# Visual-Behavior/aloception-oss

Measured on AMD Instinct MI355X. Metric: frames/sec (whole node) DeformableDETR-R50 inference, higher is better.
Workload: dtype bf16; 1 GPU; DeformableDETR-R50 inference bf16, batch 8 synthetic 1333x800 frames per GPU, random-init weights; launch=hip-graph replay + eager inference(), per_gpu_batch=8, global_batch=8, parallelism=batch-sharded x1, no collective

## Files before the change

### aloception-oss_amd/csrc/common.hpp

```cpp
#pragma once
#include <hip/hip_runtime.h>
#include <stdint.h>

#include <cstdarg>
#include <cstdio>
#include <type_traits>

#include "../../include/alo_hotpath.h"

namespace alo {

char* error_buffer();
inline int fail(alo_status_t code, const char* fmt, ...) {
    va_list ap;
    va_start(ap, fmt);
    vsnprintf(error_buffer(), 512, fmt, ap);
    va_end(ap);
    return (int)code;
}
#define ALO_REQUIRE(cond, code, ...) \
    do {                             \
        if (!(cond)) return ::alo::fail(code, __VA_ARGS__); \
    } while (0)

template <typename... P>
inline bool aligned16(const P*... p) {
    return ((... | (uintptr_t)p) & 15) == 0;
}

constexpr int kLdsLimit = 160 * 1024;
template <auto kernel>
int launch(dim3 grid, dim3 block, size_t lds, hipStream_t stream, const char* what, void** args) {
    ALO_REQUIRE(lds <= (size_t)kLdsLimit, ALO_ERR_UNSUPPORTED, "%s: %zu bytes of dynamic LDS, the limit is %d", what, lds, kLdsLimit);
    const void* fn = reinterpret_cast<const void*>(kernel);
    hipError_t e = hipSuccess;
    if (lds > 48 * 1024) {
        static unsigned long long done = 0;
        int dev = 0;
        e = hipGetDevice(&dev);
        const unsigned long long bit = 1ull << (dev & 63);
        if (e == hipSuccess && !(__atomic_load_n(&done, __ATOMIC_ACQUIRE) & bit)) {
            e = hipFuncSetAttribute(fn, hipFuncAttributeMaxDynamicSharedMemorySize, kLdsLimit);
            if (e == hipSuccess) __atomic_fetch_or(&done, bit, __ATOMIC_RELEASE);
        }
    }
    if (e == hipSuccess) e = hipLaunchKernel(fn, grid, block, args, lds, stream);
    if (e == hipSuccess) e = hipGetLastError();
    if (e != hipSuccess) return fail(ALO_ERR_LAUNCH, "%s: %s", what, hipGetErrorString(e));
    return ALO_OK;
}

constexpr int kNumXcd = 8;

__device__ __forceinline__ unsigned xcd_contiguous_block(unsigned bid, unsigned nblocks) {
    const unsigned q = nblocks / kNumXcd, r = nblocks % kNumXcd;
    const unsigned xcd = bid % kNumXcd, k = bid / kNumXcd;
    const unsigned start = xcd < r ? xcd * (q + 1) : r * (q + 1) + (xcd - r) * q;
    return start + k;
}

struct WidePlan {
    int words[31];
};
bool msda_wide_plan(int N, int S, int M, int D, int Lq, int value_dtype, const int32_t* host_shapes, WidePlan* wp);
int msda_wide_launch(const void* value, const int32_t* shapes, const int32_t* lstart, const void* loc, const void* attn,
                     const void* grad_out, void* grad_value, void* grad_loc, void* grad_attn, const WidePlan& wp, int D,
                     int value_dtype, hipStream_t stream);

struct RowGather {
    int s, Wo, HoWo, W, HW;
};
inline RowGather row_gather(int stride = 1, int Ho = 1, int Wo = 1, int H = 1, int W = 1) { return {stride, Wo, Ho * Wo, W, H * W}; }

int linear_shortk_gather(const void* x, const void* weight, const void* bias, const void* residual, void* y, long M, int N, int K,
                         int relu, const RowGather& gather, hipStream_t stream);

#define ALO_RELU_RES(fn, first, relu, residual, ...)                                                                          \
    ((residual) ? ((relu) ? fn<first, true, true>(__VA_ARGS__) : fn<first, false, true>(__VA_ARGS__))                          \
                : ((relu) ? fn<first, true, false>(__VA_ARGS__) : fn<first, false, false>(__VA_ARGS__)))

typedef __attribute__((ext_vector_type(4))) unsigned int u32x4;
typedef __attribute__((ext_vector_type(2))) unsigned int u32x2;
typedef __attribute__((ext_vector_type(4))) float f32x4;
typedef __attribute__((ext_vector_type(16))) float f32x16;

struct bf16_t {
    uint16_t bits;
};

__device__ __forceinline__ float relu_keep_nan(float v) { return (v > 0.f || v != v) ? v : 0.f; }

__device__ __forceinline__ float bf16_to_f32(uint16_t b) { return __uint_as_float(((unsigned)b) << 16); }
__device__ __forceinline__ uint16_t f32_to_bf16(float f) {
    const __bf16 b = static_cast<__bf16>(f);
    return __builtin_bit_cast(uint16_t, b);
}
__device__ __forceinline__ unsigned pack_bf16x2(float lo, float hi) {
    typedef __bf16 bf16x2_hw __attribute__((ext_vector_type(2)));
    typedef float f32x2_hw __attribute__((ext_vector_type(2)));
    const bf16x2_hw r = __builtin_convertvector(f32x2_hw{lo, hi}, bf16x2_hw);
    return __builtin_bit_cast(unsigned, r);
}

struct f16_t {
    uint16_t bits;
};
__device__ __forceinline__ float f16_to_f32(uint16_t b) { return (float)__builtin_bit_cast(_Float16, b); }
__device__ __forceinline__ uint16_t f32_to_f16(float f) {
    const _Float16 h = static_cast<_Float16>(f);
    return __builtin_bit_cast(uint16_t, h);
}
__device__ __forceinline__ unsigned pack_f16x2(float lo, float hi) {
    typedef _Float16 f16x2_hw __attribute__((ext_vector_type(2)));
    typedef float f32x2_hw __attribute__((ext_vector_type(2)));
    const f16x2_hw r = __builtin_convertvector(f32x2_hw{lo, hi}, f16x2_hw);
    return __builtin_bit_cast(unsigned, r);
}
template <typename T>
__device__ __forceinline__ void unpack2(unsigned w, float& lo, float& hi) {
    if constexpr (std::is_same<T, f16_t>::value) {
        lo = f16_to_f32((uint16_t)(w & 0xffffu));
        hi = f16_to_f32((uint16_t)(w >> 16));
    } else {
        lo = __uint_as_float(w << 16);
        hi = __uint_as_float(w & 0xffff0000u);
    }
}
template <typename T>
__device__ __forceinline__ unsigned pack2(float lo, float hi) {
    if constexpr (std::is_same<T, f16_t>::value) return pack_f16x2(lo, hi);
    else return pack_bf16x2(lo, hi);
}

typedef __attribute__((ext_vector_type(8))) __bf16 bf16x8_t;
__device__ __forceinline__ bf16x8_t as_bf16x8(const u32x4& v) {
    union { u32x4 u; bf16x8_t b; } x;
    x.u = v;
    return x.b;
}

typedef __attribute__((ext_vector_type(8))) _Float16 f16x8_t;
__device__ __forceinline__ f16x8_t as_f16x8(const u32x4& v) {
    union { u32x4 u; f16x8_t h; } x;
    x.u = v;
    return x.h;
}
template <typename T>
__device__ __forceinline__ f32x16 mfma_32x32x16(const u32x4& a, const u32x4& b, const f32x16& c) {
    if constexpr (std::is_same<T, f16_t>::value) return __builtin_amdgcn_mfma_f32_32x32x16_f16(as_f16x8(a), as_f16x8(b), c, 0, 0, 0);
    else return __builtin_amdgcn_mfma_f32_32x32x16_bf16(as_bf16x8(a), as_bf16x8(b), c, 0, 0, 0);
}

template <typename T, bool RELU>
__device__ __forceinline__ u32x4 add_residual_x8(const u32x4& v, const u32x4& rv) {
    const unsigned a4[4] = {v.x, v.y, v.z, v.w}, r4[4] = {rv.x, rv.y, rv.z, rv.w};
    unsigned o4[4];
#pragma unroll
    for (int i = 0; i < 4; ++i) {
        float alo, ahi, rlo, rhi;
        unpack2<T>(a4[i], alo, ahi);
        unpack2<T>(r4[i], rlo, rhi);
        float lo = alo + rlo, hi = ahi + rhi;
        if (RELU) { lo = relu_keep_nan(lo); hi = relu_keep_nan(hi); }
        o4[i] = pack2<T>(lo, hi);
    }
    return u32x4{o4[0], o4[1], o4[2], o4[3]};
}

__device__ __forceinline__ long gather_row(const RowGather& g, long row) {
    if (g.s <= 1) return row;
    const long n = row / g.HoWo;
    const int rem = (int)(row - n * g.HoWo);
    const int yo = rem / g.Wo, xo = rem - yo * g.Wo;
    return n * g.HW + (long)(yo * g.s) * g.W + xo * g.s;
}

__device__ __forceinline__ __amdgpu_buffer_rsrc_t make_rsrc(const void* base, unsigned bytes) {
    return __builtin_amdgcn_make_buffer_rsrc(const_cast<void*>(base), 0, (int)bytes, 0x00020000);
}
constexpr unsigned kOutOfRange = 0xC0000000u;

template <typename T, typename CT, int VEC>
struct Loader;

template <>
struct Loader<float, float, 4> {
    using raw_t = u32x4;
    static __device__ __forceinline__ raw_t load(__amdgpu_buffer_rsrc_t r, unsigned off) {
        return __builtin_amdgcn_raw_buffer_load_b128(r, off, 0, 0);
    }
    static __device__ __forceinline__ void widen(const raw_t& x, float (&v)[4]) {
        v[0] = __uint_as_float(x.x); v[1] = __uint_as_float(x.y); v[2] = __uint_as_float(x.z); v[3] = __uint_as_float(x.w);
    }
};
template <>
struct Loader<float, float, 1> {
    using raw_t = unsigned;
    static __device__ __forceinline__ raw_t load(__amdgpu_buffer_rsrc_t r, unsigned off) {
        return __builtin_amdgcn_raw_buffer_load_b32(r, off, 0, 0);
    }
    static __device__ __forceinline__ void widen(const raw_t& x, float (&v)[1]) { v[0] = __uint_as_float(x); }
};
template <>
struct Loader<double, double, 2> {
    using raw_t = u32x4;
    static __device__ __forceinline__ raw_t load(__amdgpu_buffer_rsrc_t r, unsigned off) {
        return __builtin_amdgcn_raw_buffer_load_b128(r, off, 0, 0);
    }
    static __device__ __forceinline__ void widen(const raw_t& x, double (&v)[2]) {
        v[0] = __hiloint2double((int)x.y, (int)x.x);
        v[1] = __hiloint2double((int)x.w, (int)x.z);
    }
};
template <>
struct Loader<double, double, 1> {
    using raw_t = u32x2;
    static __device__ __forceinline__ raw_t load(__amdgpu_buffer_rsrc_t r, unsigned off) {
        return __builtin_amdgcn_raw_buffer_load_b64(r, off, 0, 0);
    }
    static __device__ __forceinline__ void widen(const raw_t& x, double (&v)[1]) {
        v[0] = __hiloint2double((int)x.y, (int)x.x);
    }
};
template <>
struct Loader<bf16_t, float, 8> {
    using raw_t = u32x4;
    static __device__ __forceinline__ raw_t load(__amdgpu_buffer_rsrc_t r, unsigned off) {
        return __builtin_amdgcn_raw_buffer_load_b128(r, off, 0, 0);
    }
    static __device__ __forceinline__ void widen(const raw_t& x, float (&v)[8]) {
        const unsigned w[4] = {x.x, x.y, x.z, x.w};
#pragma unroll
        for (int i = 0; i < 4; ++i) {
            v[2 * i] = __uint_as_float(w[i] << 16);
            v[2 * i + 1] = __uint_as_float(w[i] & 0xffff0000u);
        }
    }
};
template <>
struct Loader<bf16_t, float, 1> {
    using raw_t = unsigned short;
    static __device__ __forceinline__ raw_t load(__amdgpu_buffer_rsrc_t r, unsigned off) {
        return __builtin_amdgcn_raw_buffer_load_b16(r, off, 0, 0);
    }
    static __device__ __forceinline__ void widen(const raw_t& x, float (&v)[1]) { v[0] = bf16_to_f32(x); }
};

template <>
struct Loader<f16_t, float, 8> {
    using raw_t = u32x4;
    static __device__ __forceinline__ raw_t load(__amdgpu_buffer_rsrc_t r, unsigned off) {
        return __builtin_amdgcn_raw_buffer_load_b128(r, off, 0, 0);
    }
    static __device__ __forceinline__ void widen(const raw_t& x, float (&v)[8]) {
        const unsigned w[4] = {x.x, x.y, x.z, x.w};
#pragma unroll
        for (int i = 0; i < 4; ++i) unpack2<f16_t>(w[i], v[2 * i], v[2 * i + 1]);
    }
};
template <>
struct Loader<f16_t, float, 1> {
    using raw_t = unsigned short;
    static __device__ __forceinline__ raw_t load(__amdgpu_buffer_rsrc_t r, unsigned off) {
        return __builtin_amdgcn_raw_buffer_load_b16(r, off, 0, 0);
    }
    static __device__ __forceinline__ void widen(const raw_t& x, float (&v)[1]) { v[0] = f16_to_f32(x); }
};

__device__ __forceinline__ float ld(const float* p) { return *p; }
__device__ __forceinline__ double ld(const double* p) { return *p; }
__device__ __forceinline__ float ld(const bf16_t* p) { return bf16_to_f32(p->bits); }
__device__ __forceinline__ float ld(const f16_t* p) { return f16_to_f32(p->bits); }
__device__ __forceinline__ void st(float* p, float v) { *p = v; }
__device__ __forceinline__ void st(double* p, double v) { *p = v; }
__device__ __forceinline__ void st(bf16_t* p, float v) { p->bits = f32_to_bf16(v); }
__device__ __forceinline__ void st(f16_t* p, float v) { p->bits = f32_to_f16(v); }

template <typename T, typename CT, int VEC>
__device__ __forceinline__ void store_vec(T* p, const CT (&v)[VEC]) {
    if constexpr (sizeof(T) == 4 && VEC == 4) {
        *reinterpret_cast<f32x4*>(p) = f32x4{(float)v[0], (float)v[1], (float)v[2], (float)v[3]};
    } else if constexpr (sizeof(T) == 8 && VEC == 2) {
        *reinterpret_cast<double2*>(p) = double2{(double)v[0], (double)v[1]};
    } else if constexpr (sizeof(T) == 2 && VEC == 8) {
        u32x4 o;
        o.x = pack2<T>(v[0], v[1]);
        o.y = pack2<T>(v[2], v[3]);
        o.z = pack2<T>(v[4], v[5]);
        o.w = pack2<T>(v[6], v[7]);
        *reinterpret_cast<u32x4*>(p) = o;
    } else {
#pragma unroll
        for (int i = 0; i < VEC; ++i) st(p + i, v[i]);
    }
}

__device__ __forceinline__ float wave_sum(float v) {
#pragma unroll
    for (int o = 32; o > 0; o >>= 1) v += __shfl_xor(v, o, 64);
    return v;
}

constexpr int kTileRows = 64;
constexpr int kTileStride = 256 * 2 + 16;
constexpr int kTileKB = 2;
constexpr int kTileBatches = 16 / kTileKB;

template <typename T>
__device__ __forceinline__ void load_batch(u32x4 (&buf)[2][kTileKB], const T* frag0, size_t tile_stride, int batch) {
#pragma unroll
    for (int t = 0; t < 2; ++t)
#pragma unroll
        for (int j = 0; j < kTileKB; ++j)
            buf[t][j] = *reinterpret_cast<const u32x4*>(frag0 + t * tile_stride + (size_t)(kTileKB * batch + j) * 512);
    __builtin_amdgcn_sched_barrier(0);
}
template <typename T = bf16_t>
__device__ __forceinline__ void mma_batch(f32x16 (&acc)[2][2], const unsigned char* a_lds, const u32x4 (&buf)[2][kTileKB], int batch,
                                          int nl, int kg) {
    u32x4 af[2][kTileKB];
#pragma unroll
    for (int j = 0; j < kTileKB; ++j) {
        const int s = kTileKB * batch + j;
        af[0][j] = *reinterpret_cast<const u32x4*>(a_lds + nl * kTileStride + (16 * s + 8 * kg) * 2);
        af[1][j] = *reinterpret_cast<const u32x4*>(a_lds + (32 + nl) * kTileStride + (16 * s + 8 * kg) * 2);
    }
#pragma unroll
    for (int j = 0; j < kTileKB; ++j) {
        const u32x4 a0 = af[0][j], a1 = af[1][j];
        acc[0][0] = mfma_32x32x16<T>(buf[0][j], a0, acc[0][0]);
        acc[0][1] = mfma_32x32x16<T>(buf[1][j], a0, acc[0][1]);
        acc[1][0] = mfma_32x32x16<T>(buf[0][j], a1, acc[1][0]);
        acc[1][1] = mfma_32x32x16<T>(buf[1][j], a1, acc[1][1]);
    }
    __builtin_amdgcn_sched_barrier(0);
}
template <typename T>
__device__ __forceinline__ void mma_tile256(f32x16 (&acc)[2][2], const unsigned char* a_lds, u32x4 (&bufa)[2][kTileKB],
                                            u32x4 (&bufb)[2][kTileKB], const T* w, size_t tile_stride, const T* next,
                                            size_t next_stride, int nl, int kg) {
#pragma unroll
    for (int bt = 0; bt < kTileBatches; bt += 2) {
        load_batch(bufb, w, tile_stride, bt + 1);
        mma_batch<T>(acc, a_lds, bufa, bt, nl, kg);
        if (bt + 2 < kTileBatches) load_batch(bufa, w, tile_stride, bt + 2);
        else if (next != nullptr) load_batch(bufa, next, next_stride, 0);
        mma_batch<T>(acc, a_lds, bufb, bt + 1, nl, kg);
    }
}

template <typename T>
__device__ __forceinline__ void fetch_tile256(u32x4 (&v)[8], const T* X, long row0, long M, int tid) {
#pragma unroll
    for (int j = 0; j < 8; ++j) {
        const int p = tid + 256 * j;
        long row = row0 + (p >> 5);
        row = row < M ? row : M - 1;
        v[j] = *reinterpret_cast<const u32x4*>(X + row * 256 + (p & 31) * 8);
    }
}
__device__ __forceinline__ void park_tile256(unsigned char* lds, const u32x4 (&v)[8], int tid) {
#pragma unroll
    for (int j = 0; j < 8; ++j) {
        const int p = tid + 256 * j;
        *reinterpret_cast<u32x4*>(lds + (p >> 5) * kTileStride + (p & 31) * 16) = v[j];
    }
}
template <bool ADD_BIAS, bool RELU, typename T = bf16_t>
__device__ __forceinline__ void stage_tile256(unsigned char* lds, const f32x16 (&acc)[2][2], const float* bias, int wave, int nl, int kg) {
#pragma unroll
    for (int t = 0; t < 2; ++t)
#pragma unroll
        for (int q = 0; q < 4; ++q) {
            const int col = 64 * wave + 32 * t + 8 * q + 4 * kg;
            f32x4 bb = {0.f, 0.f, 0.f, 0.f};
            if constexpr (ADD_BIAS) bb = *reinterpret_cast<const f32x4*>(bias + col);
#pragma unroll
            for (int a = 0; a < 2; ++a) {
                float v0 = acc[a][t][4 * q], v1 = acc[a][t][4 * q + 1], v2 = acc[a][t][4 * q + 2], v3 = acc[a][t][4 * q + 3];
                if constexpr (ADD_BIAS) { v0 += bb[0]; v1 += bb[1]; v2 += bb[2]; v3 += bb[3]; }
                if constexpr (RELU) { v0 = relu_keep_nan(v0); v1 = relu_keep_nan(v1); v2 = relu_keep_nan(v2); v3 = relu_keep_nan(v3); }
                *reinterpret_cast<u32x2*>(lds + (32 * a + nl) * kTileStride + col * 2) = u32x2{pack2<T>(v0, v1), pack2<T>(v2, v3)};
            }
        }
}

}
```

### aloception-oss_amd/csrc/gemm.hip

```cpp
#include "common.hpp"

namespace alo {
namespace {

constexpr int kRows = 64;
constexpr int kOutStride = 64 * 2 + 16;

struct GemmDims {
    long M;
    int N;
    int tiles;
    int S;
    RowGather g;
};

template <typename T, int kK, bool RELU, bool HAS_RES, bool HM>
__global__ void __launch_bounds__(256, 2)
linear_shortk_kernel(const T* __restrict__ X, const T* __restrict__ W, const T* __restrict__ bias,
                     const T* __restrict__ R, T* __restrict__ Y, const GemmDims dm) {
    constexpr int kRowBytes = kK * 2 + 16;
    constexpr int kSteps = kK / 16;
    constexpr int kPieces = kK / 8;
    constexpr int kLoads = kRows * kPieces / 256;
    static_assert(kRows * kPieces % 256 == 0, "the tile loader gives every thread the same number of pieces");
    extern __shared__ __attribute__((aligned(16))) unsigned char smem[];
    unsigned char* const xbuf = smem;
    const int tid = threadIdx.x, wave = tid >> 6, lane = tid & 63;
    unsigned char* obuf = smem + kRows * kRowBytes + wave * (kRows * kOutStride);

    const int col0 = blockIdx.y * 256 + wave * 64;
    const bool has_cols = col0 < dm.N;
    const int nl = lane & 31, kg = lane >> 5;

    u32x4 wreg[2][kSteps];
    float* const bias_tab = reinterpret_cast<float*>(smem + kRows * kRowBytes + 4 * (kRows * kOutStride)) + wave * 64;
    if (has_cols) {
#pragma unroll
        for (int t = 0; t < 2; ++t) {
            const T* wr = W + (size_t)(col0 + 32 * t + nl) * kK + 8 * kg;
#pragma unroll
            for (int s = 0; s < kSteps; ++s) wreg[t][s] = *reinterpret_cast<const u32x4*>(wr + 16 * s);
        }
        const int r = lane & 15, t = (lane >> 4) & 1, k2 = lane >> 5;
        bias_tab[lane] = bias != nullptr ? ld(&bias[col0 + 32 * t + (r & 3) + 8 * (r >> 2) + 4 * k2]) : 0.f;
    }

    auto fetch = [&](int tile, u32x4 (&r)[kLoads]) {
#pragma unroll
        for (int j = 0; j < kLoads; ++j) {
            const int p = tid + 256 * j;
            long row = (long)tile * kRows + p / kPieces;
            row = gather_row(dm.g, row < dm.M ? row : dm.M - 1);
            r[j] = *reinterpret_cast<const u32x4*>(X + row * kK + (p % kPieces) * 8);
        }
    };
    auto park = [&](const u32x4 (&r)[kLoads]) {
#pragma unroll
        for (int j = 0; j < kLoads; ++j) {
            const int p = tid + 256 * j;
            *reinterpret_cast<u32x4*>(xbuf + (p / kPieces) * kRowBytes + (p % kPieces) * 16) = r[j];
        }
    };

    int tile = blockIdx.x;
    if (tile >= dm.tiles) return;
    u32x4 stage[kLoads];
    fetch(tile, stage);

    for (;;) {
        park(stage);
        __syncthreads();
        const int next = tile + gridDim.x;
        const bool more = next < dm.tiles;
        if (more) fetch(next, stage);

        if (has_cols) {
#pragma unroll
            for (int half = 0; half < kRows / 32; ++half) {
                f32x16 acc[2];
#pragma unroll
                for (int t = 0; t < 2; ++t)
#pragma unroll
                    for (int q = 0; q < 4; ++q) {
                        const f32x4 b4 = *reinterpret_cast<const f32x4*>(bias_tab + (kg * 2 + t) * 16 + 4 * q);
#pragma unroll
                        for (int i = 0; i < 4; ++i) acc[t][4 * q + i] = b4[i];
                    }
#pragma unroll
                for (int s = 0; s < kSteps; ++s) {
                    const u32x4 a = *reinterpret_cast<const u32x4*>(xbuf + (32 * half + nl) * kRowBytes + (16 * s + 8 * kg) * 2);
                    acc[0] = mfma_32x32x16<T>(wreg[0][s], a, acc[0]);
                    acc[1] = mfma_32x32x16<T>(wreg[1][s], a, acc[1]);
                }
#pragma unroll
                for (int t = 0; t < 2; ++t)
#pragma unroll
                    for (int q = 0; q < 4; ++q) {
                        float v0 = acc[t][4 * q], v1 = acc[t][4 * q + 1], v2 = acc[t][4 * q + 2], v3 = acc[t][4 * q + 3];
                        if (RELU && !HAS_RES) { v0 = relu_keep_nan(v0); v1 = relu_keep_nan(v1); v2 = relu_keep_nan(v2); v3 = relu_keep_nan(v3); }
                        *reinterpret_cast<u32x2*>(obuf + (32 * half + nl) * kOutStride + (32 * t + 8 * q + 4 * kg) * 2) =
                            u32x2{pack2<T>(v0, v1), pack2<T>(v2, v3)};
                    }
            }
            __builtin_amdgcn_fence(__ATOMIC_RELEASE, "wavefront");
            __builtin_amdgcn_wave_barrier();
            __builtin_amdgcn_fence(__ATOMIC_ACQUIRE, "wavefront");
            if constexpr (HM) {
                const unsigned char* mask = reinterpret_cast<const unsigned char*>(R);
                const int heads = dm.N / 32;
#pragma unroll
                for (int hh = 0; hh < 2; ++hh) {
#pragma unroll
                    for (int pass = 0; pass < kRows / 16; ++pass) {
                        const int row = pass * 16 + (lane >> 2);
                        const long grow = (long)tile * kRows + row;
                        if (grow < dm.M) {
                            u32x4 v = *reinterpret_cast<const u32x4*>(obuf + row * kOutStride + hh * 64 + (lane & 3) * 16);
                            if (mask != nullptr && mask[grow]) v = u32x4{0u, 0u, 0u, 0u};
                            const long nb = grow / dm.S, sp = grow - nb * dm.S;
                            const int head = col0 / 32 + hh;
                            *reinterpret_cast<u32x4*>(Y + ((nb * heads + head) * dm.S + sp) * 32 + (lane & 3) * 8) = v;
                        }
                    }
                }
            } else
#pragma unroll
            for (int pass = 0; pass < kRows / 8; ++pass) {
                const int row = pass * 8 + (lane >> 3);
                const long grow = (long)tile * kRows + row;
                u32x4 v = *reinterpret_cast<const u32x4*>(obuf + row * kOutStride + (lane & 7) * 16);
                if (grow < dm.M) {
                    if constexpr (HAS_RES) {
                        v = add_residual_x8<T, RELU>(v, *reinterpret_cast<const u32x4*>(R + grow * dm.N + col0 + (lane & 7) * 8));
                    }
                    *reinterpret_cast<u32x4*>(Y + grow * dm.N + col0 + (lane & 7) * 8) = v;
                }
            }
        }
        if (!more) break;
        __syncthreads();
        tile = next;
    }
}

}
}

using namespace alo;

namespace {
template <typename T, int kK>
struct ShortK {
    using type = T;
    static constexpr int K = kK;
};

template <class Cfg, bool RELU, bool HAS_RES, bool HM = false>
int launch_shortk(const void* x, const void* weight, const void* bias, const void* residual, void* y, long M, int N,
                  hipStream_t stream, int S = 0, const RowGather& gather = row_gather()) {
    GemmDims dm;
    dm.M = M; dm.N = N; dm.tiles = (int)((M + kRows - 1) / kRows); dm.S = S; dm.g = gather;
    constexpr int K = Cfg::K;
    const size_t lds = kRows * (K * 2 + 16) + 4 * kRows * kOutStride + 4 * 64 * sizeof(float);
    const int cols = (N + 255) / 256;
    int gx = 512 / cols;
    if (gx > dm.tiles) gx = dm.tiles;
    if (gx < 1) gx = 1;
    void* args[] = {&x, &weight, &bias, &residual, &y, &dm};
    return launch<linear_shortk_kernel<typename Cfg::type, K, RELU, HAS_RES, HM>>(dim3(gx, cols), 256, lds, stream, "alo_linear_shortk", args);
}

template <typename T>
int dispatch_shortk(const void* x, const void* weight, const void* bias, const void* residual, void* y, long M, int N, int K, int relu,
                    const RowGather& gather, hipStream_t stream) {
    using K64 = ShortK<T, 64>;
    using K128 = ShortK<T, 128>;
    using K256 = ShortK<T, 256>;
    if (K == 64) return ALO_RELU_RES(launch_shortk, K64, relu, residual, x, weight, bias, residual, y, M, N, stream, 0, gather);
    if (K == 128) return ALO_RELU_RES(launch_shortk, K128, relu, residual, x, weight, bias, residual, y, M, N, stream, 0, gather);
    if (K == 256) return ALO_RELU_RES(launch_shortk, K256, relu, residual, x, weight, bias, residual, y, M, N, stream, 0, gather);
    return fail(ALO_ERR_UNSUPPORTED, "alo_conv1x1_nhwc: the resident-weight kernel needs Cin in (64, 128, 256), got %d", K);
}
}

extern "C" int alo_linear_shortk(const void* x, const void* weight, const void* bias, const void* residual, void* y, long M,
                                 int N, int K, int relu, int dtype, void* stream) {
    ALO_REQUIRE(dtype == ALO_BF16 || dtype == ALO_F16, ALO_ERR_UNSUPPORTED, "alo_linear_shortk: bf16 / fp16 only (dtype %d)", dtype);
    ALO_REQUIRE(x && weight && y, ALO_ERR_INVALID_ARGUMENT, "alo_linear_shortk: null pointer argument");
    ALO_REQUIRE(M > 0 && N > 0 && N % 64 == 0, ALO_ERR_INVALID_ARGUMENT,
                "alo_linear_shortk: M must be positive and N a positive multiple of 64 (M=%ld N=%d)", M, N);
    ALO_REQUIRE(K == 64 || K == 128 || K == 256, ALO_ERR_UNSUPPORTED, "alo_linear_shortk: K must be 64, 128 or 256, got %d", K);
    ALO_REQUIRE(aligned16(x, weight, y, residual), ALO_ERR_INVALID_ARGUMENT, "alo_linear_shortk: pointers must be 16-byte aligned");
    hipStream_t st = static_cast<hipStream_t>(stream);
    if (dtype == ALO_F16) return dispatch_shortk<f16_t>(x, weight, bias, residual, y, M, N, K, relu, row_gather(), st);
    return dispatch_shortk<bf16_t>(x, weight, bias, residual, y, M, N, K, relu, row_gather(), st);
}

int alo::linear_shortk_gather(const void* x, const void* weight, const void* bias, const void* residual, void* y, long M, int N, int K,
                              int relu, const RowGather& gather, hipStream_t stream) {
    return dispatch_shortk<bf16_t>(x, weight, bias, residual, y, M, N, K, relu, gather, stream);
}

namespace alo {
namespace {

constexpr int kFfnRows = kTileRows;
constexpr int kFfnStride = kTileStride;

struct FfnDims {
    long M;
    int F;
    int tiles;
};

template <typename T>
__global__ void __launch_bounds__(256, 2)
ffn256_kernel(const T* __restrict__ X, const T* __restrict__ W1, const T* __restrict__ B1,
              const T* __restrict__ W2, const T* __restrict__ B2, T* __restrict__ Y, const FfnDims dm) {
    extern __shared__ __attribute__((aligned(16))) unsigned char smem[];
    unsigned char* const xs = smem;
    unsigned char* const hs = smem + kFfnRows * kFfnStride;
    const int tid = threadIdx.x, wave = tid >> 6, lane = tid & 63;
    const int nl = lane & 31, kg = lane >> 5;
    const int F = dm.F;

    float* const b1s = reinterpret_cast<float*>(smem + 2 * kFfnRows * kFfnStride);
    float* const b2s = b1s + F;
    for (int i = tid; i < F; i += 256) b1s[i] = B1 ? ld(B1 + i) : 0.f;
    b2s[tid] = B2 ? ld(B2 + tid) : 0.f;

    const int fs = F / 16;
    auto w1_frag = [&](int r0) { return W1 + ((size_t)((r0 + 64 * wave) / 32) * 16 * 64 + lane) * 8; };
    auto w2_frag = [&](int r0) { return W2 + (((size_t)(2 * wave) * fs + r0 / 16) * 64 + lane) * 8; };

    for (int tile = blockIdx.x; tile < dm.tiles; tile += gridDim.x) {
        {
            u32x4 xv[8];
            fetch_tile256(xv, X, (long)tile * kFfnRows, dm.M, tid);
            park_tile256(xs, xv, tid);
        }
        u32x4 bufa[2][kTileKB], bufb[2][kTileKB];
        load_batch(bufa, w1_frag(0), (size_t)16 * 512, 0);
        __syncthreads();

        f32x16 acc2[2][2];
#pragma unroll
        for (int a = 0; a < 2; ++a)
#pragma unroll
            for (int t = 0; t < 2; ++t)
#pragma unroll
                for (int i = 0; i < 16; ++i) acc2[a][t][i] = 0.f;

        for (int r0 = 0; r0 < F; r0 += 256) {
            f32x16 acc1[2][2];
#pragma unroll
            for (int a = 0; a < 2; ++a)
#pragma unroll
                for (int t = 0; t < 2; ++t)
#pragma unroll
                    for (int i = 0; i < 16; ++i) acc1[a][t][i] = 0.f;
            const T* w1p = w1_frag(r0);
            const T* w2p = w2_frag(r0);
            mma_tile256(acc1, xs, bufa, bufb, w1p, (size_t)16 * 512, w2p, (size_t)fs * 512, nl, kg);
            stage_tile256<true, true, T>(hs, acc1, b1s + r0, wave, nl, kg);
            __syncthreads();

            mma_tile256(acc2, hs, bufa, bufb, w2p, (size_t)fs * 512, r0 + 256 < F ? w1_frag(r0 + 256) : nullptr, (size_t)16 * 512, nl, kg);
            __syncthreads();
        }

        stage_tile256<true, false, T>(hs, acc2, b2s, wave, nl, kg);
        __syncthreads();
#pragma unroll
        for (int j = 0; j < 8; ++j) {
            const int p = tid + 256 * j;
            const long row = (long)tile * kFfnRows + (p >> 5);
            if (row < dm.M)
                *reinterpret_cast<u32x4*>(Y + row * 256 + (p & 31) * 8) =
                    *reinterpret_cast<const u32x4*>(hs + (p >> 5) * kFfnStride + (p & 31) * 16);
        }
        __syncthreads();
    }
}

}
}

namespace alo {
namespace {
__global__ void __launch_bounds__(256)
pack_mfma_b_kernel(const bf16_t* __restrict__ W, bf16_t* __restrict__ P, int N, int K) {
    const long total = (long)N * K / 8;
    for (long i = (long)blockIdx.x * 256 + threadIdx.x; i < total; i += (long)gridDim.x * 256) {
        const int lane = (int)(i % 64);
        const long frag = i / 64;
        const int s = (int)(frag % (K / 16)), t = (int)(frag / (K / 16));
        const int n = 32 * t + (lane & 31), k = 16 * s + 8 * (lane >> 5);
        *reinterpret_cast<u32x4*>(P + i * 8) = *reinterpret_cast<const u32x4*>(W + (size_t)n * K + k);
    }
}
}
}

extern "C" int alo_pack_mfma_b(const void* w, void* packed, int N, int K, int dtype, void* stream) {
    ALO_REQUIRE(dtype == ALO_BF16 || dtype == ALO_F16, ALO_ERR_UNSUPPORTED, "alo_pack_mfma_b: bf16 / fp16 only (dtype %d)", dtype);
    ALO_REQUIRE(w && packed, ALO_ERR_INVALID_ARGUMENT, "alo_pack_mfma_b: null pointer argument");
    ALO_REQUIRE(N > 0 && K > 0 && N % 32 == 0 && K % 16 == 0, ALO_ERR_INVALID_ARGUMENT,
                "alo_pack_mfma_b: N must be a multiple of 32 and K a multiple of 16 (N=%d K=%d)", N, K);
    long total = (long)N * K / 8;
    unsigned blocks = (unsigned)((total + 255) / 256 > 4096 ? 4096 : (total + 255) / 256);
    void* args[] = {&w, &packed, &N, &K};
    return launch<pack_mfma_b_kernel>(blocks, 256, 0, static_cast<hipStream_t>(stream), "alo_pack_mfma_b", args);
}

extern "C" int alo_ffn256(const void* x, const void* w1, const void* b1, const void* w2, const void* b2, void* y, long M,
                          int F, int dtype, void* stream) {
    ALO_REQUIRE(dtype == ALO_BF16 || dtype == ALO_F16, ALO_ERR_UNSUPPORTED, "alo_ffn256: bf16 / fp16 only (dtype %d)", dtype);
    ALO_REQUIRE(x && w1 && w2 && y, ALO_ERR_INVALID_ARGUMENT, "alo_ffn256: null pointer argument");
    ALO_REQUIRE(M > 0 && F > 0 && F % 256 == 0, ALO_ERR_INVALID_ARGUMENT,
                "alo_ffn256: M must be positive and the hidden width a positive multiple of 256 (M=%ld F=%d)", M, F);
    ALO_REQUIRE(aligned16(x, w1, w2, y), ALO_ERR_INVALID_ARGUMENT, "alo_ffn256: pointers must be 16-byte aligned");
    FfnDims dm;
    dm.M = M; dm.F = F; dm.tiles = (int)((M + kFfnRows - 1) / kFfnRows);
    const size_t lds = 2 * kFfnRows * kFfnStride + ((size_t)F + 256) * sizeof(float);
    int gx = dm.tiles < 512 ? dm.tiles : 512;
    void* args[] = {&x, &w1, &b1, &w2, &b2, &y, &dm};
    if (lds > (size_t)kLdsLimit) return fail(ALO_ERR_UNSUPPORTED, "alo_ffn256: hidden width %d needs %zu bytes of LDS", F, lds);
    if (dtype == ALO_F16) return launch<ffn256_kernel<f16_t>>(gx, 256, lds, static_cast<hipStream_t>(stream), "alo_ffn256", args);
    return launch<ffn256_kernel<bf16_t>>(gx, 256, lds, static_cast<hipStream_t>(stream), "alo_ffn256", args);
}

extern "C" int alo_value_proj_head_major(const void* x, const void* weight, const void* bias, const void* padding_mask,
                                         void* value_hm, int batch, int S, int heads, int K, int dtype, void* stream) {
    ALO_REQUIRE(dtype == ALO_BF16 || dtype == ALO_F16, ALO_ERR_UNSUPPORTED, "alo_value_proj_head_major: bf16 / fp16 only (dtype %d)", dtype);
    ALO_REQUIRE(x && weight && value_hm, ALO_ERR_INVALID_ARGUMENT, "alo_value_proj_head_major: null pointer argument");
    ALO_REQUIRE(batch > 0 && S > 0 && heads > 0 && heads % 2 == 0, ALO_ERR_INVALID_ARGUMENT,
                "alo_value_proj_head_major: batch, S must be positive and the head count even (batch=%d S=%d heads=%d)", batch, S,
                heads);
    ALO_REQUIRE(K == 64 || K == 128 || K == 256, ALO_ERR_UNSUPPORTED, "alo_value_proj_head_major: K must be 64, 128 or 256, got %d", K);
    ALO_REQUIRE(aligned16(x, weight, value_hm), ALO_ERR_INVALID_ARGUMENT, "alo_value_proj_head_major: pointers must be 16-byte aligned");
    hipStream_t st = static_cast<hipStream_t>(stream);
    const long M = (long)batch * S;
    const int N = heads * 32;
    if (dtype == ALO_F16) {
        if (K == 64) return launch_shortk<ShortK<f16_t, 64>, false, false, true>(x, weight, bias, padding_mask, value_hm, M, N, st, S);
        if (K == 128) return launch_shortk<ShortK<f16_t, 128>, false, false, true>(x, weight, bias, padding_mask, value_hm, M, N, st, S);
        return launch_shortk<ShortK<f16_t, 256>, false, false, true>(x, weight, bias, padding_mask, value_hm, M, N, st, S);
    }
    if (K == 64) return launch_shortk<ShortK<bf16_t, 64>, false, false, true>(x, weight, bias, padding_mask, value_hm, M, N, st, S);
    if (K == 128) return launch_shortk<ShortK<bf16_t, 128>, false, false, true>(x, weight, bias, padding_mask, value_hm, M, N, st, S);
    return launch_shortk<ShortK<bf16_t, 256>, false, false, true>(x, weight, bias, padding_mask, value_hm, M, N, st, S);
}
```

Before: 904.6 frames/s.

## Add few-rows FFN kernel with deep weight prefetch ring for small M

Adds a second fused FFN kernel that uses 32-row tiles and a configurable ring of weight-fragment register buffers (default 8 deep). The host picks it when M is at most 64 rows per CU, and an environment variable can force either path. The shared MMA helpers are generalised over row-tile count and ring depth. The aim is to spread small-M FFN work (such as the decoder's 8x300 queries) over more CUs and hide weight-load latency. The cost is lower MFMA reuse per weight load and much higher register pressure, with one wave group per CU.

```diff
diff --git a/aloception-oss_amd/csrc/common.hpp b/aloception-oss_amd/csrc/common.hpp
--- a/aloception-oss_amd/csrc/common.hpp
+++ b/aloception-oss_amd/csrc/common.hpp
@@ -315,59 +315,75 @@
             buf[t][j] = *reinterpret_cast<const u32x4*>(frag0 + t * tile_stride + (size_t)(kTileKB * batch + j) * 512);
     __builtin_amdgcn_sched_barrier(0);
 }
-template <typename T = bf16_t>
-__device__ __forceinline__ void mma_batch(f32x16 (&acc)[2][2], const unsigned char* a_lds, const u32x4 (&buf)[2][kTileKB], int batch,
+template <typename T = bf16_t, int RT>
+__device__ __forceinline__ void mma_batch(f32x16 (&acc)[RT][2], const unsigned char* a_lds, const u32x4 (&buf)[2][kTileKB], int batch,
                                           int nl, int kg) {
-    u32x4 af[2][kTileKB];
+    u32x4 af[RT][kTileKB];
 #pragma unroll
     for (int j = 0; j < kTileKB; ++j) {
         const int s = kTileKB * batch + j;
         af[0][j] = *reinterpret_cast<const u32x4*>(a_lds + nl * kTileStride + (16 * s + 8 * kg) * 2);
-        af[1][j] = *reinterpret_cast<const u32x4*>(a_lds + (32 + nl) * kTileStride + (16 * s + 8 * kg) * 2);
-    }
-#pragma unroll
-    for (int j = 0; j < kTileKB; ++j) {
-        const u32x4 a0 = af[0][j], a1 = af[1][j];
-        acc[0][0] = mfma_32x32x16<T>(buf[0][j], a0, acc[0][0]);
-        acc[0][1] = mfma_32x32x16<T>(buf[1][j], a0, acc[0][1]);
-        acc[1][0] = mfma_32x32x16<T>(buf[0][j], a1, acc[1][0]);
-        acc[1][1] = mfma_32x32x16<T>(buf[1][j], a1, acc[1][1]);
-    }
+        if constexpr (RT == 2) af[1][j] = *reinterpret_cast<const u32x4*>(a_lds + (32 + nl) * kTileStride + (16 * s + 8 * kg) * 2);
+    }
+#pragma unroll
+    for (int j = 0; j < kTileKB; ++j)
+#pragma unroll
+        for (int a = 0; a < RT; ++a) {
+            acc[a][0] = mfma_32x32x16<T>(buf[0][j], af[a][j], acc[a][0]);
+            acc[a][1] = mfma_32x32x16<T>(buf[1][j], af[a][j], acc[a][1]);
+        }
     __builtin_amdgcn_sched_barrier(0);
 }
-template <typename T>
-__device__ __forceinline__ void mma_tile256(f32x16 (&acc)[2][2], const unsigned char* a_lds, u32x4 (&bufa)[2][kTileKB],
+template <typename T, int RT, int NB>
+__device__ __forceinline__ void mma_ring256(f32x16 (&acc)[RT][2], const unsigned char* a_lds, u32x4 (*const (&ring)[NB])[kTileKB],
+                                            const T* w, size_t tile_stride, const T* next, size_t next_stride, int nl, int kg) {
+    static_assert(NB >= 2 && kTileBatches % NB == 0, "the ring must divide the batches of one contraction");
+    typedef u32x4 (&buf_t)[2][kTileKB];
+#pragma unroll
+    for (int bt = 0; bt < kTileBatches; ++bt) {
+        const int ahead = bt + NB - 1;
+        if (ahead < kTileBatches) load_batch(reinterpret_cast<buf_t>(*ring[ahead % NB]), w, tile_stride, ahead);
+        else if (next != nullptr) load_batch(reinterpret_cast<buf_t>(*ring[ahead % NB]), next, next_stride, ahead - kTileBatches);
+        mma_batch<T>(acc, a_lds, reinterpret_cast<buf_t>(*ring[bt % NB]), bt, nl, kg);
+    }
+}
+template <typename T, int RT>
+__device__ __forceinline__ void mma_tile256(f32x16 (&acc)[RT][2], const unsigned char* a_lds, u32x4 (&bufa)[2][kTileKB],
                                             u32x4 (&bufb)[2][kTileKB], const T* w, size_t tile_stride, const T* next,
                                             size_t next_stride, int nl, int kg) {
-#pragma unroll
-    for (int bt = 0; bt < kTileBatches; bt += 2) {
-        load_batch(bufb, w, tile_stride, bt + 1);
-        mma_batch<T>(acc, a_lds, bufa, bt, nl, kg);
-        if (bt + 2 < kTileBatches) load_batch(bufa, w, tile_stride, bt + 2);
-        else if (next != nullptr) load_batch(bufa, next, next_stride, 0);
-        mma_batch<T>(acc, a_lds, bufb, bt + 1, nl, kg);
-    }
-}
-
-template <typename T>
-__device__ __forceinline__ void fetch_tile256(u32x4 (&v)[8], const T* X, long row0, long M, int tid) {
-#pragma unroll
-    for (int j = 0; j < 8; ++j) {
+    u32x4 (*const ring[2])[kTileKB] = {bufa, bufb};
+    mma_ring256(acc, a_lds, ring, w, tile_stride, next, next_stride, nl, kg);
+}
+template <typename T, int RT, int NB>
+__device__ __forceinline__ void mma_tile256(f32x16 (&acc)[RT][2], const unsigned char* a_lds, u32x4 (&bufs)[NB][2][kTileKB], const T* w,
+                                            size_t tile_stride, const T* next, size_t next_stride, int nl, int kg) {
+    u32x4 (*ring[NB])[kTileKB];
+#pragma unroll
+    for (int b = 0; b < NB; ++b) ring[b] = bufs[b];
+    u32x4 (*const (&cring)[NB])[kTileKB] = ring;
+    mma_ring256(acc, a_lds, cring, w, tile_stride, next, next_stride, nl, kg);
+}
+
+template <typename T, int NP>
+__device__ __forceinline__ void fetch_tile256(u32x4 (&v)[NP], const T* X, long row0, long M, int tid) {
+#pragma unroll
+    for (int j = 0; j < NP; ++j) {
         const int p = tid + 256 * j;
         long row = row0 + (p >> 5);
         row = row < M ? row : M - 1;
         v[j] = *reinterpret_cast<const u32x4*>(X + row * 256 + (p & 31) * 8);
     }
 }
-__device__ __forceinline__ void park_tile256(unsigned char* lds, const u32x4 (&v)[8], int tid) {
-#pragma unroll
-    for (int j = 0; j < 8; ++j) {
+template <int NP>
+__device__ __forceinline__ void park_tile256(unsigned char* lds, const u32x4 (&v)[NP], int tid) {
+#pragma unroll
+    for (int j = 0; j < NP; ++j) {
         const int p = tid + 256 * j;
         *reinterpret_cast<u32x4*>(lds + (p >> 5) * kTileStride + (p & 31) * 16) = v[j];
     }
 }
-template <bool ADD_BIAS, bool RELU, typename T = bf16_t>
-__device__ __forceinline__ void stage_tile256(unsigned char* lds, const f32x16 (&acc)[2][2], const float* bias, int wave, int nl, int kg) {
+template <bool ADD_BIAS, bool RELU, typename T = bf16_t, int RT>
+__device__ __forceinline__ void stage_tile256(unsigned char* lds, const f32x16 (&acc)[RT][2], const float* bias, int wave, int nl, int kg) {
 #pragma unroll
     for (int t = 0; t < 2; ++t)
 #pragma unroll
@@ -376,7 +392,7 @@
             f32x4 bb = {0.f, 0.f, 0.f, 0.f};
             if constexpr (ADD_BIAS) bb = *reinterpret_cast<const f32x4*>(bias + col);
 #pragma unroll
-            for (int a = 0; a < 2; ++a) {
+            for (int a = 0; a < RT; ++a) {
                 float v0 = acc[a][t][4 * q], v1 = acc[a][t][4 * q + 1], v2 = acc[a][t][4 * q + 2], v3 = acc[a][t][4 * q + 3];
                 if constexpr (ADD_BIAS) { v0 += bb[0]; v1 += bb[1]; v2 += bb[2]; v3 += bb[3]; }
                 if constexpr (RELU) { v0 = relu_keep_nan(v0); v1 = relu_keep_nan(v1); v2 = relu_keep_nan(v2); v3 = relu_keep_nan(v3); }
diff --git a/aloception-oss_amd/csrc/gemm.hip b/aloception-oss_amd/csrc/gemm.hip
--- a/aloception-oss_amd/csrc/gemm.hip
+++ b/aloception-oss_amd/csrc/gemm.hip
@@ -1,4 +1,7 @@
 #include "common.hpp"
+
+#include <cstdlib>
+#include <cstring>
 
 namespace alo {
 namespace {
@@ -283,6 +286,84 @@
     }
 }
 
+constexpr int kFewRows = 32;
+#ifndef ALO_FFN_FEW_RING
+#define ALO_FFN_FEW_RING 8
+#endif
+constexpr int kFewRing = ALO_FFN_FEW_RING;
+
+template <typename T>
+__global__ void __launch_bounds__(256, 1)
+ffn256_few_rows_kernel(const T* __restrict__ X, const T* __restrict__ W1, const T* __restrict__ B1,
+                       const T* __restrict__ W2, const T* __restrict__ B2, T* __restrict__ Y, const FfnDims dm) {
+    extern __shared__ __attribute__((aligned(16))) unsigned char smem[];
+    unsigned char* const xs = smem;
+    unsigned char* const hs = smem + kFewRows * kFfnStride;
+    const int tid = threadIdx.x, wave = tid >> 6, lane = tid & 63;
+    const int nl = lane & 31, kg = lane >> 5;
+    const int F = dm.F;
+
+    const int fs = F / 16;
+    auto w1_frag = [&](int r0) { return W1 + ((size_t)((r0 + 64 * wave) / 32) * 16 * 64 + lane) * 8; };
+    auto w2_frag = [&](int r0) { return W2 + (((size_t)(2 * wave) * fs + r0 / 16) * 64 + lane) * 8; };
+    u32x4 ring[kFewRing][2][kTileKB];
+#pragma unroll
+    for (int b = 0; b < kFewRing - 1; ++b) load_batch(ring[b], w1_frag(0), (size_t)16 * 512, b);
+
+    float* const b1s = reinterpret_cast<float*>(smem + 2 * kFewRows * kFfnStride);
+    float* const b2s = b1s + F;
+    for (int i = tid; i < F; i += 256) b1s[i] = B1 ? ld(B1 + i) : 0.f;
+    b2s[tid] = B2 ? ld(B2 + tid) : 0.f;
+
+    for (int tile = blockIdx.x; tile < dm.tiles; tile += gridDim.x) {
+        {
+            u32x4 xv[kFewRows / 8];
+            fetch_tile256(xv, X, (long)tile * kFewRows, dm.M, tid);
+            park_tile256(xs, xv, tid);
+        }
+        __syncthreads();
+
+        f32x16 acc2[1][2];
+#pragma unroll
+        for (int t = 0; t < 2; ++t)
+#pragma unroll
+            for (int i = 0; i < 16; ++i) acc2[0][t][i] = 0.f;
+
+        for (int r0 = 0; r0 < F; r0 += 256) {
+            f32x16 acc1[1][2];
+#pragma unroll
+            for (int t = 0; t < 2; ++t)
+#pragma unroll
+                for (int i = 0; i < 16; ++i) acc1[0][t][i] = 0.f;
+            const T* w1p = w1_frag(r0);
+            const T* w2p = w2_frag(r0);
+            __builtin_assume(w2p != nullptr);
+            mma_tile256(acc1, xs, ring, w1p, (size_t)16 * 512, w2p, (size_t)fs * 512, nl, kg);
+            stage_tile256<true, true, T>(hs, acc1, b1s + r0, wave, nl, kg);
+            __syncthreads();
+            const T* w1n = w1_frag(r0 + 256 < F ? r0 + 256 : 0);
+            __builtin_assume(w1n != nullptr);
+            mma_tile256(acc2, hs, ring, w2p, (size_t)fs * 512, w1n, (size_t)16 * 512, nl, kg);
+            __syncthreads();
+        }
+
+        stage_tile256<true, false, T>(hs, acc2, b2s, wave, nl, kg);
+        __syncthreads();
+#pragma unroll
+        for (int j = 0; j < kFewRows / 8; ++j) {
+            const int p = tid + 256 * j;
+            const long row = (long)tile * kFewRows + (p >> 5);
+            if (row < dm.M)
+                *reinterpret_cast<u32x4*>(Y + row * 256 + (p & 31) * 8) =
+                    *reinterpret_cast<const u32x4*>(hs + (p >> 5) * kFfnStride + (p & 31) * 16);
+        }
+        __syncthreads();
+    }
+}
+
+constexpr long kFewRowsPerCu = 64;
+inline bool ffn_few_rows(long M, int cus) { return M <= kFewRowsPerCu * cus; }
+
 }
 }
 
@@ -320,14 +401,28 @@
     ALO_REQUIRE(M > 0 && F > 0 && F % 256 == 0, ALO_ERR_INVALID_ARGUMENT,
                 "alo_ffn256: M must be positive and the hidden width a positive multiple of 256 (M=%ld F=%d)", M, F);
     ALO_REQUIRE(aligned16(x, w1, w2, y), ALO_ERR_INVALID_ARGUMENT, "alo_ffn256: pointers must be 16-byte aligned");
+    if (2 * kFfnRows * kFfnStride + ((size_t)F + 256) * sizeof(float) > (size_t)kLdsLimit)
+        return fail(ALO_ERR_UNSUPPORTED, "alo_ffn256: hidden width %d needs %zu bytes of LDS", F,
+                    2 * kFfnRows * kFfnStride + ((size_t)F + 256) * sizeof(float));
+    hipStream_t st = static_cast<hipStream_t>(stream);
+    int dev = 0, cus = 0;
+    if (hipGetDevice(&dev) != hipSuccess || hipDeviceGetAttribute(&cus, hipDeviceAttributeMultiprocessorCount, dev) != hipSuccess || cus < 1)
+        return fail(ALO_ERR_LAUNCH, "alo_ffn256: cannot read the device's compute unit count");
+    const char* knob = getenv("ALO_FFN256");
+    const bool few = knob && !strcmp(knob, "few") ? true : knob && !strcmp(knob, "stream") ? false : ffn_few_rows(M, cus);
+    const int rows = few ? kFewRows : kFfnRows;
     FfnDims dm;
-    dm.M = M; dm.F = F; dm.tiles = (int)((M + kFfnRows - 1) / kFfnRows);
-    const size_t lds = 2 * kFfnRows * kFfnStride + ((size_t)F + 256) * sizeof(float);
-    int gx = dm.tiles < 512 ? dm.tiles : 512;
+    dm.M = M; dm.F = F; dm.tiles = (int)((M + rows - 1) / rows);
+    const size_t lds = 2 * rows * kFfnStride + ((size_t)F + 256) * sizeof(float);
+    const int cap = few ? cus : 512;
+    int gx = dm.tiles < cap ? dm.tiles : cap;
     void* args[] = {&x, &w1, &b1, &w2, &b2, &y, &dm};
-    if (lds > (size_t)kLdsLimit) return fail(ALO_ERR_UNSUPPORTED, "alo_ffn256: hidden width %d needs %zu bytes of LDS", F, lds);
-    if (dtype == ALO_F16) return launch<ffn256_kernel<f16_t>>(gx, 256, lds, static_cast<hipStream_t>(stream), "alo_ffn256", args);
-    return launch<ffn256_kernel<bf16_t>>(gx, 256, lds, static_cast<hipStream_t>(stream), "alo_ffn256", args);
+    if (few) {
+        if (dtype == ALO_F16) return launch<ffn256_few_rows_kernel<f16_t>>(gx, 256, lds, st, "alo_ffn256", args);
+        return launch<ffn256_few_rows_kernel<bf16_t>>(gx, 256, lds, st, "alo_ffn256", args);
+    }
+    if (dtype == ALO_F16) return launch<ffn256_kernel<f16_t>>(gx, 256, lds, st, "alo_ffn256", args);
+    return launch<ffn256_kernel<bf16_t>>(gx, 256, lds, st, "alo_ffn256", args);
 }
 
 extern "C" int alo_value_proj_head_major(const void* x, const void* weight, const void* bias, const void* padding_mask,
```

Result: no change. 909.2 frames/s (median of 2 runs) (+0.5%).
